# autonomousvision/connecting_the_dots

Measured on AMD Instinct MI355X. Metric: Mpix*disparities/s on 512x432x128 cost volume; disparity MAE vs ref, higher is better.
Workload: dtype f32

## Files before the change

### connecting_the_dots_amd/csrc/argmax_rerank.hip

```cpp
#include "ctd_internal.h"
#include "ctd_ncc_point.h"
#include "ctd_rank.h"
#include "ctd_tail.h"


namespace ctd {

constexpr int kScanBatch = 8;
template <int PX>
__global__ __launch_bounds__(256) __attribute__((amdgpu_waves_per_eu(5, 8))) void argmax_scan_kernel(const float* __restrict__ vol, int64_t* __restrict__ idx,
                                                          float* __restrict__ best, int D, long HW, int W,
                                                          int bs, float eps, long total_threads, WorkList work) {
  const long t = (long)blockIdx.x * blockDim.x + threadIdx.x;
  if (t >= total_threads) return;
  const long p0 = t * PX;
  const long f = p0 / HW, q0 = p0 - f * HW;
  const float* v = vol + f * D * HW + q0;
  const int w0 = (int)(q0 % W);
  float v0[PX], v1[PX];
  int i0[PX], dc[PX];
#pragma unroll
  for (int k = 0; k < PX; ++k) { v0[k] = -INFINITY; v1[k] = -INFINITY; i0[k] = 0; dc[k] = w0 + k + (bs - 1 - bs / 2); }
  constexpr int kBatch = kScanBatch;
  const bool wave_masks = __any(dc[0] < D - 1);
  for (int d0 = 0; d0 < D; d0 += kBatch) {
    float x[kBatch][PX];
#pragma unroll
    for (int u = 0; u < kBatch; ++u) {
      const float* src = v + (long)min(d0 + u, D - 1) * HW;
      if constexpr (PX == 4) {
        typedef float f4 __attribute__((ext_vector_type(4)));
        const f4 q = __builtin_nontemporal_load((const f4*)src);
        x[u][0] = q.x; x[u][1] = q.y; x[u][2] = q.z; x[u][3] = q.w;
      } else if constexpr (PX == 2) {
        typedef float f2 __attribute__((ext_vector_type(2)));
        const f2 q = __builtin_nontemporal_load((const f2*)src);
        x[u][0] = q.x; x[u][1] = q.y;
      } else {
        x[u][0] = __builtin_nontemporal_load(src);
      }
    }
    if (wave_masks || d0 + kBatch > D) {
#pragma unroll
      for (int u = 0; u < kBatch; ++u) {
        const int d = d0 + u;
#pragma unroll
        for (int k = 0; k < PX; ++k) {
          const float y = (d > dc[k] || d >= D) ? -INFINITY : x[u][k];
          v1[k] = __builtin_amdgcn_fmed3f(v0[k], v1[k], y);
          i0[k] = y > v0[k] ? d : i0[k];
          v0[k] = fmaxf(v0[k], y);
        }
      }
    } else {
#pragma unroll
      for (int u = 0; u < kBatch; ++u) {
#pragma unroll
        for (int k = 0; k < PX; ++k) {
          const float y = x[u][k];
          v1[k] = __builtin_amdgcn_fmed3f(v0[k], v1[k], y);
          i0[k] = y > v0[k] ? d0 + u : i0[k];
          v0[k] = fmaxf(v0[k], y);
        }
      }
    }
  }
#pragma unroll
  for (int k = 0; k < PX; ++k) {
    const bool hard = v1[k] >= v0[k] - eps;
    idx[p0 + k] = hard ? (int64_t)(-1 - i0[k]) : (int64_t)i0[k];
    if (best) best[p0 + k] = v0[k];
    if (hard) work.list[atomicAdd(work.counters, 1u)] = p0 + k;
  }
}

constexpr int kMaskWords = 8;

__device__ inline float wave_maxf(float v) {
#pragma unroll
  for (int o = 32; o > 0; o >>= 1) v = fmaxf(v, __shfl_xor(v, o));
  return v;
}

struct RunSource {
  const float* run_vals;
  const float* v1;
  int W1, xoff, per_frame;
};

template <int WORDS, bool VOL>
__device__ __forceinline__ void resolve_role(float* lds_resolve, const float* __restrict__ vol, const float* __restrict__ in0,
                                             const float* __restrict__ in1, long in1_frame_stride,
                                             int64_t* __restrict__ idx, float* __restrict__ best, int D, int H, int W, int bs,
                                             float eps, WorkList work, RunSource rsrc, unsigned role_block,
                                             unsigned n_role_blocks, unsigned waves_used = 4, unsigned* stamp = nullptr) {
  if ((threadIdx.x >> 6) >= waves_used) return;
  const int lane = threadIdx.x & 63;
  const int half = bs / 2, span = bs + D - 1;
  float* sA = lds_resolve + (threadIdx.x >> 6) * 2 * (bs * bs + bs * span);
  float* sB = sA + bs * bs;
  float* sAq = sB + bs * span;
  float* sBq = sAq + bs * bs;
  const float bs2f = (float)(bs * bs);
  const long HW = (long)H * W;
  unsigned seg_cnt[kWorkListParts];
  unsigned longest = 0;
#pragma unroll
  for (int k = 0; k < kWorkListParts; ++k) seg_cnt[k] = work.counters[min(k, work.parts - 1) * kWorkListStride];
#pragma unroll
  for (int k = 0; k < kWorkListParts; ++k) {
    if (k >= work.parts) seg_cnt[k] = 0u;
    longest = max(longest, seg_cnt[k]);
  }
  const unsigned n_slots = longest * (unsigned)work.parts;
  CTD_POST_STAMP_S(stamp, 1, longest);
  const unsigned n_waves = n_role_blocks * waves_used;
  for (unsigned slot = role_block * waves_used + (threadIdx.x >> 6); slot < n_slots; slot += n_waves) {
    const unsigned seg = slot & (unsigned)(work.parts - 1), entry = slot / (unsigned)work.parts;
    unsigned cnt = 0;
#pragma unroll
    for (int k = 0; k < kWorkListParts; ++k) cnt = seg == (unsigned)k ? seg_cnt[k] : cnt;
    if (entry >= cnt) continue;
    const long pj = work.list[(long)seg * work.seg_cap + entry];
    CTD_POST_STAMP_S(stamp, 2, pj);
    CTD_POST_STAMP_ITEM(stamp);
    const long fj = pj / HW, qj = pj - fj * HW;
    const int hj = (int)(qj / W), wj = (int)(qj - (long)hj * W);
    const float* v = VOL ? vol + fj * D * HW + qj : nullptr;
    const int d_clamped = wj + (bs - 1 - bs / 2);
    unsigned long long mask[WORDS];
    int n_cand = 0;
    float x[WORDS];
    bool run_listed = false;
    float rv = 0.f;
    if constexpr (VOL) {
      if (rsrc.run_vals && d_clamped < D) {
        const long z = rsrc.per_frame ? fj : 0;
        run_listed = rsrc.v1[(z * H + hj) * rsrc.W1 + (rsrc.xoff - (bs - 1 - bs / 2))] == 0.f;
        if (run_listed) rv = rsrc.run_vals[(fj * H + hj) * D + d_clamped];
      }
#pragma unroll
      for (int wd = 0; wd < WORDS; ++wd) {
        const int d = min(wd * 64 + lane, D - 1);
        x[wd] = v[(long)(rsrc.run_vals ? min(d, d_clamped) : d) * HW];
        if (run_listed && d >= d_clamped) x[wd] = rv;
      }
      CTD_POST_STAMP_V(stamp, 3, x[0]);
    }
    constexpr int kPreA = 2, kPreB = 20;
    const bool pre = !VOL && bs * bs <= 64 * kPreA && bs * span <= 64 * kPreB;
    const float* a = in0 + fj * HW;
    const float* b = in1 + fj * in1_frame_stride;
    float ta[kPreA], tb[kPreB];
    if (pre) {
#pragma unroll
      for (int k = 0; k < kPreA; ++k) {
        const int i = min(lane + 64 * k, bs * bs - 1);
        const int bh = i / bs, bw = i - bh * bs;
        ta[k] = a[(long)clampi(hj + bh - half, 0, H - 1) * W + clampi(wj + bw - half, 0, W - 1)];
      }
#pragma unroll
      for (int k = 0; k < kPreB; ++k) {
        const int i = min(lane + 64 * k, bs * span - 1);
        const int bh = i / span, c = i - bh * span;
        tb[k] = b[(long)clampi(hj + bh - half, 0, H - 1) * W + clampi(wj - half - (D - 1) + c, 0, W - 1)];
      }
    }
    if constexpr (VOL) {
      float m = -INFINITY;
#pragma unroll
      for (int wd = 0; wd < WORDS; ++wd)
        if (wd * 64 + lane < D && wd * 64 + lane <= d_clamped) m = fmaxf(m, x[wd]);
      m = wave_maxf(m);
      bool have_clamped = false;
#pragma unroll
      for (int wd = 0; wd < WORDS; ++wd) {
        unsigned long long bits = __ballot(wd * 64 + lane < D && x[wd] >= m - eps);
        const int c0 = d_clamped - wd * 64;
        if (c0 < 64) {
          const unsigned long long run = c0 <= 0 ? bits : bits & ~((1ull << c0) - 1ull);
          bits &= ~run;
          if (!have_clamped && run) {
            bits |= run & (0ull - run);
            have_clamped = true;
          }
        }
        mask[wd] = bits;
        n_cand += __popcll(bits);
      }
    } else {
#pragma unroll
      for (int wd = 0; wd < WORDS; ++wd) {
        const int last = min(D - 1, d_clamped) - wd * 64;
        mask[wd] = last < 0 ? 0ull : (last >= 63 ? ~0ull : ((1ull << (last + 1)) - 1ull));
        n_cand += __popcll(mask[wd]);
      }
    }
    float eb = 0.f;
    int ei = 0x7fffffff;
    const bool rescore = VOL ? n_cand > 1 : n_cand >= 1;
    if (rescore && pre) {
#pragma unroll
      for (int k = 0; k < kPreA; ++k)
        if (lane + 64 * k < bs * bs) {
          sA[lane + 64 * k] = ta[k];
          sAq[lane + 64 * k] = ta[k] / bs2f;
        }
#pragma unroll
      for (int k = 0; k < kPreB; ++k)
        if (lane + 64 * k < bs * span) {
          sB[lane + 64 * k] = tb[k];
          sBq[lane + 64 * k] = tb[k] / bs2f;
        }
    } else if (rescore) {
      for (int i = lane; i < bs * bs; i += 64) {
        const int bh = i / bs, bw = i - bh * bs;
        const float xa = a[(long)clampi(hj + bh - half, 0, H - 1) * W + clampi(wj + bw - half, 0, W - 1)];
        sA[i] = xa;
        sAq[i] = xa / bs2f;
      }
      constexpr int NB = 20;
      for (int i0 = lane; i0 < bs * span; i0 += 64 * NB) {
        float t[NB];
#pragma unroll
        for (int k = 0; k < NB; ++k) {
          const int i = min(i0 + 64 * k, bs * span - 1);
          const int bh = i / span, c = i - bh * span;
          t[k] = b[(long)clampi(hj + bh - half, 0, H - 1) * W + clampi(wj - half - (D - 1) + c, 0, W - 1)];
        }
#pragma unroll
        for (int k = 0; k < NB; ++k)
          if (i0 + 64 * k < bs * span) {
            sB[i0 + 64 * k] = t[k];
            sBq[i0 + 64 * k] = t[k] / bs2f;
          }
      }
    }
    CTD_POST_STAMP(stamp, 4);
    if (rescore) {
      for (int c0 = 0; c0 < n_cand; c0 += 64) {
        int my_d = -1, k = 0;
#pragma unroll
        for (int wd = 0; wd < WORDS; ++wd) {
          unsigned long long mj = mask[wd];
          if (k + __popcll(mj) <= c0 || k >= c0 + 64) { k += __popcll(mj); continue; }
          while (mj) {
            const int d = wd * 64 + __ffsll((long long)mj) - 1;
            mj &= mj - 1;
            if (k - c0 == lane) my_d = d;
            ++k;
          }
        }
        float e = -INFINITY;
        if (my_d >= 0) e = bs == 9 ? ncc_exact_point_lds_bs<9>(sA, sB, sAq, sBq, span, (D - 1) - my_d)
                                   : ncc_exact_point_lds(sA, sB, bs, span, (D - 1) - my_d);
        const float em = wave_maxf(e);
        const unsigned long long holders = __ballot(my_d >= 0 && e == em);
        const int dl = __shfl(my_d, holders ? __ffsll((long long)holders) - 1 : 0);
        if (ei == 0x7fffffff || em > eb) { eb = em; ei = dl; }
      }
    } else {
#pragma unroll
      for (int wd = 0; wd < WORDS; ++wd)
        if (mask[wd]) ei = min(ei, wd * 64 + __ffsll((long long)mask[wd]) - 1);
    }
    CTD_POST_STAMP_S(stamp, 5, ei);
    if (lane == 0) {
      idx[pj] = ei;
      if (best) {
        if constexpr (VOL) best[pj] = (run_listed && ei >= d_clamped) ? rv : v[(long)(rsrc.run_vals ? min(ei, d_clamped) : ei) * HW];
        else if (rescore) best[pj] = eb;
      }
    }
    CTD_POST_STAMP(stamp, 6);
    CTD_POST_STAMP(stamp, 9);
    stamp = nullptr;
  }
}

template <int WORDS, bool VOL>
__global__ __launch_bounds__(256) void argmax_resolve_kernel(const float* __restrict__ vol, const float* __restrict__ in0,
                                                             const float* __restrict__ in1, long in1_frame_stride,
                                                             int64_t* __restrict__ idx, float* __restrict__ best, int D,
                                                             int H, int W, int bs, float eps, WorkList work) {
  extern __shared__ float lds_dyn[];
  resolve_role<WORDS, VOL>(lds_dyn, vol, in0, in1, in1_frame_stride, idx, best, D, H, W, bs, eps, work,
                           RunSource{nullptr, nullptr, 0, 0, 0}, blockIdx.x, gridDim.x);
}

constexpr long kResolveBlocks = 1024;
constexpr unsigned kTailResolveWaves = 2;

template <int WORDS, bool VOL>
__global__ __launch_bounds__(256) void rank_tail_kernel(float* __restrict__ vol, const float* __restrict__ in0,
                                                        const float* __restrict__ in1, long in1_frame_stride,
                                                        int64_t* __restrict__ idx, float* __restrict__ best,
                                                        const unsigned char* __restrict__ flags, int frames, int D, int H,
                                                        int W, int bs, float eps, WorkList work, RunSource rsrc,
                                                        unsigned* __restrict__ counters,
                                                        const unsigned long long* __restrict__ run_rows,
                                                        const unsigned long long* __restrict__ flag_a,
                                                        const unsigned long long* __restrict__ flag_b, unsigned n_resolve,
                                                        unsigned n_runs, unsigned n_decode) {
  extern __shared__ float lds_dyn[];
  const unsigned n_pair = min(n_resolve, n_runs);
  unsigned role, rb;
  if (blockIdx.x < n_decode) { role = 2; rb = blockIdx.x; }
  else {
    const unsigned b = blockIdx.x - n_decode;
    if (b < 2 * n_pair) { role = b & 1; rb = b >> 1; }
    else { role = n_resolve > n_runs ? 0 : 1; rb = b - n_pair; }
  }
  if (blockIdx.x == 0 && threadIdx.x == 0) counters[0] = 0u;
  unsigned* stamp = CTD_POST_STAMP_SLOT(role);
  if (role == 0) {
    resolve_role<WORDS, VOL>(lds_dyn, vol, in0, in1, in1_frame_stride, idx, best, D, H, W, bs, eps, work, rsrc, rb, n_resolve,
                             kTailResolveWaves, stamp);
  } else if (role == 1) {
    if constexpr (VOL)
      runs_role(vol, rsrc.run_vals, counters, run_rows, rsrc.per_frame, 1, H, W, D, bs, (int)(rb >> 2), (int)(rb & 3), 4,
                (int*)lds_dyn, stamp);
  } else {
    decode_role((unsigned long long*)idx, best, flags, counters, flag_a, flag_b, rsrc.per_frame, frames, H, W, D,
                rb * 4 + (threadIdx.x >> 6), n_decode * 4, stamp);
  }
}


CTD_POST_STAMP_EXPORT(ctd_debug_read_tail_stamps)

template <bool VOL>
static int launch_resolve(const float* vol, const float* in0, const float* in1, long in1_frame_stride, int64_t* idx,
                          float* best, long total, int D, int H, int W, int bs, float eps, const WorkList& work,
                          hipStream_t stream) {
  const size_t lds = sizeof(float) * 4 * 2 * ((size_t)bs * bs + (size_t)bs * (bs + D - 1));
  if (lds > 160 * 1024) return CTD_ERR_UNSUPPORTED;
  const long chunks = (total + 255) / 256;
  auto resolve = D <= 128 ? argmax_resolve_kernel<2, VOL> : (D <= 256 ? argmax_resolve_kernel<4, VOL> : argmax_resolve_kernel<8, VOL>);
  if (lds > 64 * 1024)
    CTD_HIP_TRY(hipFuncSetAttribute((const void*)resolve, hipFuncAttributeMaxDynamicSharedMemorySize, (int)lds));
  hipLaunchKernelGGL(resolve, dim3((unsigned)(chunks < kResolveBlocks ? chunks : kResolveBlocks)), dim3(256), lds, stream, vol,
                     in0, in1, in1_frame_stride, idx, best, D, H, W, bs, eps, work);
  CTD_LAUNCH_CHECK();
  return CTD_OK;
}

template <bool VOL>
static int launch_tail(const RankPlan& rp, float* vol, const float* in0, const float* in1, long in1_frame_stride,
                       int64_t* idx, float* best, int frames, int D, int H, int W, int bs, hipStream_t stream) {
  size_t lds = sizeof(float) * kTailResolveWaves * 2 * ((size_t)bs * bs + (size_t)bs * (bs + D - 1));
  if (lds < sizeof(int) * (size_t)H) lds = sizeof(int) * (size_t)H;
  if (lds > 160 * 1024) return CTD_ERR_UNSUPPORTED;
  const long total = (long)frames * H * W;
  const long chunks = (total + 255) / 256;
  const unsigned n_resolve = rp.eps >= 0.f ? (unsigned)(chunks < kResolveBlocks ? chunks : kResolveBlocks) : 0u;
  const unsigned n_runs = VOL ? (unsigned)(frames * ceil_div(D, kRunPlanes)) * 4u : 0u;
  const unsigned n_decode = 128u;
  auto kern = D <= 128 ? rank_tail_kernel<2, VOL> : (D <= 256 ? rank_tail_kernel<4, VOL> : rank_tail_kernel<8, VOL>);
  if (lds > 64 * 1024)
    CTD_HIP_TRY(hipFuncSetAttribute((const void*)kern, hipFuncAttributeMaxDynamicSharedMemorySize, (int)lds));
  const RunSource rsrc = {rp.run_vals, rp.v1, rp.W1, rp.xoff, in1_frame_stride != 0 ? 1 : 0};
  hipLaunchKernelGGL(kern, dim3(n_resolve + n_runs + n_decode), dim3(256), lds, stream, vol, in0, in1, in1_frame_stride, idx,
                     best, rp.flags, frames, D, H, W, bs, rp.eps, rp.work, rsrc, rp.counters, rp.run_rows, rp.flag_a, rp.flag_b,
                     n_resolve,
                     n_runs, n_decode);
  CTD_LAUNCH_CHECK();
  return CTD_OK;
}

int rank_tail_f32(const RankPlan& rp, float* vol, const float* in0, const float* in1, long in1_frame_stride, int64_t* idx,
                  float* best, int frames, int D, int H, int W, int bs, hipStream_t stream) {
  return vol ? launch_tail<true>(rp, vol, in0, in1, in1_frame_stride, idx, best, frames, D, H, W, bs, stream)
             : launch_tail<false>(rp, nullptr, in0, in1, in1_frame_stride, idx, best, frames, D, H, W, bs, stream);
}

int argmax_rerank_f32(const float* vol, const float* in0, const float* in1, long in1_frame_stride, int64_t* idx,
                      float* best, int frames, int D, int H, int W, int bs, float eps, void* workspace,
                      size_t workspace_bytes, bool counter_cleared, hipStream_t stream) {
  if (D > kMaskWords * 64) return CTD_ERR_UNSUPPORTED;
  const long total = (long)frames * H * W;
  const long HW = (long)H * W;
  if (!workspace || workspace_bytes < 16 + sizeof(int64_t) * (size_t)total) return CTD_ERR_WORKSPACE;
  unsigned* n_hard = (unsigned*)workspace;
  const WorkList work = {n_hard, (int64_t*)((char*)workspace + 16), 1, W, total};
  if (!counter_cleared) CTD_HIP_TRY(hipMemsetAsync(n_hard, 0, 16, stream));
  const bool vec4 = W % 4 == 0 && ((uintptr_t)vol % 16) == 0;
  const int px = vec4 ? 4 : 1;
  if (px == 4)
    hipLaunchKernelGGL(argmax_scan_kernel<4>, dim3((unsigned)((total / 4 + 255) / 256)), dim3(256), 0, stream, vol,
                       idx, best, D, HW, W, bs, eps, total / 4, work);
  else
    hipLaunchKernelGGL(argmax_scan_kernel<1>, dim3((unsigned)((total + 255) / 256)), dim3(256), 0, stream, vol, idx,
                       best, D, HW, W, bs, eps, total, work);
  CTD_LAUNCH_CHECK();
  if (eps < 0.f) return CTD_OK;
  return launch_resolve<true>(vol, in0, in1, in1_frame_stride, idx, best, total, D, H, W, bs, eps, work, stream);
}

}
```

### connecting_the_dots_amd/csrc/ctd_ncc_point.h

```cpp
#ifndef CTD_NCC_POINT_H
#define CTD_NCC_POINT_H
#include "ctd_common.h"

namespace ctd {

__device__ inline float ncc_norm(float s0, float s1) {
  return (float)((double)sqrtf(s0 * s1) + 1e-8);
}
__device__ inline double ncc_norm(double s0, double s1) { return sqrt(s0 * s1) + 1e-8; }

__device__ inline float ncc_exact_term_lds(const float* sA, const float* sB, int bs, int span, int off) {
  const float bs2 = (float)(bs * bs);
  float mu0 = 0.f, mu1 = 0.f;
  for (int bh = 0; bh < bs; ++bh)
    for (int bw = 0; bw < bs; ++bw) {
      mu0 += sA[bh * bs + bw] / bs2;
      mu1 += sB[bh * span + bw + off] / bs2;
    }
  float s0 = 0.f, s1 = 0.f, dot = 0.f;
  for (int bh = 0; bh < bs; ++bh)
    for (int bw = 0; bw < bs; ++bw) {
      const float v0 = sA[bh * bs + bw] - mu0;
      const float v1 = sB[bh * span + bw + off] - mu1;
      dot += v0 * v1;
      s0 += v0 * v0;
      s1 += v1 * v1;
    }
  return dot / ncc_norm(s0, s1);
}
__device__ inline float ncc_exact_point_lds(const float* sA, const float* sB, int bs, int span, int off) {
  float val = 0.f;
  val += ncc_exact_term_lds(sA, sB, bs, span, off);
  return val;
}

template <int BS>
__device__ inline float ncc_exact_point_lds_bs(const float* sA, const float* sB, const float* sAq, const float* sBq,
                                               int span, int off) {
  float mu0 = 0.f, mu1 = 0.f;
  for (int bh = 0; bh < BS; ++bh) {
    float a[BS], b[BS];
#pragma unroll
    for (int bw = 0; bw < BS; ++bw) { a[bw] = sAq[bh * BS + bw]; b[bw] = sBq[bh * span + bw + off]; }
#pragma unroll
    for (int bw = 0; bw < BS; ++bw) {
      mu0 += a[bw];
      mu1 += b[bw];
    }
  }
  float s0 = 0.f, s1 = 0.f, dot = 0.f;
  for (int bh = 0; bh < BS; ++bh) {
    float a[BS], b[BS];
#pragma unroll
    for (int bw = 0; bw < BS; ++bw) { a[bw] = sA[bh * BS + bw]; b[bw] = sB[bh * span + bw + off]; }
#pragma unroll
    for (int bw = 0; bw < BS; ++bw) {
      const float v0 = a[bw] - mu0;
      const float v1 = b[bw] - mu1;
      dot += v0 * v1;
      s0 += v0 * v0;
      s1 += v1 * v1;
    }
  }
  float val = 0.f;
  val += dot / ncc_norm(s0, s1);
  return val;
}

}
#endif
```

Measured before the change: 1.034 million.

## Specialize bs=9 rerank path with halved LDS, two-pass means, occupancy-sized grid

Adds a bs=9 specialization of the resolve role. It stages window tiles in LDS once and runs the rescoring in two passes: a first pass computes the means from quotient-scaled values, then the raw values are restaged for the correlation sums. This halves the per-wave LDS footprint. The float divide by 81 is replaced with a reciprocal-multiply plus FMA correction, with a range guard and a fallback to true division. Work-item indices and the frame and row arithmetic are made wave-uniform via readfirstlane, which moves them to scalar registers. The tail kernel now uses 4 resolve waves with a launch-bounds occupancy hint and sizes its resolve grid from the queried occupancy. The rewrite adds complexity, and restaging between the passes costs extra LDS traffic.

```diff
diff --git a/connecting_the_dots_amd/csrc/argmax_rerank.hip b/connecting_the_dots_amd/csrc/argmax_rerank.hip
--- a/connecting_the_dots_amd/csrc/argmax_rerank.hip
+++ b/connecting_the_dots_amd/csrc/argmax_rerank.hip
@@ -1,5 +1,6 @@
 #include "ctd_internal.h"
 #include "ctd_ncc_point.h"
+#include "ctd_quot.h"
 #include "ctd_rank.h"
 #include "ctd_tail.h"
 
@@ -88,44 +89,65 @@
   int W1, xoff, per_frame;
 };
 
-template <int WORDS, bool VOL>
+constexpr int kResolveRegsA = 2, kResolveRegsB = 20;
+__host__ __device__ inline bool resolve_fits_regs(int bs, int D) {
+  return bs * bs <= 64 * kResolveRegsA && bs * (bs + D - 1) <= 64 * kResolveRegsB;
+}
+
+template <bool NARROW>
+__device__ __forceinline__ float frame_elem(const float* frame, int i) {
+  if constexpr (NARROW) return *(const float*)((const char*)frame + (unsigned)i * 4u);
+  else return frame[i];
+}
+
+inline bool resolve_b9(int bs, int D, int H, int W) { return bs == 9 && D >= 56 && D <= 128 && (long)H * W < (1L << 30); }
+
+__host__ __device__ inline int resolve_lds_floats(bool b9, int bs, int D) {
+  return b9 ? 64 * (kResolveRegsA + kResolveRegsB) : bs * bs + bs * (bs + D - 1);
+}
+
+template <int WORDS, bool VOL, bool B9>
 __device__ __forceinline__ void resolve_role(float* lds_resolve, const float* __restrict__ vol, const float* __restrict__ in0,
                                              const float* __restrict__ in1, long in1_frame_stride,
-                                             int64_t* __restrict__ idx, float* __restrict__ best, int D, int H, int W, int bs,
+                                             int64_t* __restrict__ idx, float* __restrict__ best, int D, int H, int W, int bs_rt,
                                              float eps, WorkList work, RunSource rsrc, unsigned role_block,
                                              unsigned n_role_blocks, unsigned waves_used = 4, unsigned* stamp = nullptr) {
   if ((threadIdx.x >> 6) >= waves_used) return;
   const int lane = threadIdx.x & 63;
+  const int bs = B9 ? 9 : bs_rt;
   const int half = bs / 2, span = bs + D - 1;
-  float* sA = lds_resolve + (threadIdx.x >> 6) * 2 * (bs * bs + bs * span);
-  float* sB = sA + bs * bs;
-  float* sAq = sB + bs * span;
-  float* sBq = sAq + bs * bs;
+  float* sA = lds_resolve + (threadIdx.x >> 6) * resolve_lds_floats(B9, bs, D);
+  float* sB = sA + (B9 ? 64 * kResolveRegsA : bs * bs);
   const float bs2f = (float)(bs * bs);
   const long HW = (long)H * W;
-  unsigned seg_cnt[kWorkListParts];
   unsigned longest = 0;
-#pragma unroll
-  for (int k = 0; k < kWorkListParts; ++k) seg_cnt[k] = work.counters[min(k, work.parts - 1) * kWorkListStride];
-#pragma unroll
-  for (int k = 0; k < kWorkListParts; ++k) {
-    if (k >= work.parts) seg_cnt[k] = 0u;
-    longest = max(longest, seg_cnt[k]);
+  {
+    unsigned seg_cnt[kWorkListParts];
+#pragma unroll
+    for (int k = 0; k < kWorkListParts; ++k) seg_cnt[k] = work.counters[min(k, work.parts - 1) * kWorkListStride];
+#pragma unroll
+    for (int k = 0; k < kWorkListParts; ++k)
+      if (k < work.parts) longest = max(longest, seg_cnt[k]);
   }
   const unsigned n_slots = longest * (unsigned)work.parts;
   CTD_POST_STAMP_S(stamp, 1, longest);
   const unsigned n_waves = n_role_blocks * waves_used;
   for (unsigned slot = role_block * waves_used + (threadIdx.x >> 6); slot < n_slots; slot += n_waves) {
     const unsigned seg = slot & (unsigned)(work.parts - 1), entry = slot / (unsigned)work.parts;
-    unsigned cnt = 0;
-#pragma unroll
-    for (int k = 0; k < kWorkListParts; ++k) cnt = seg == (unsigned)k ? seg_cnt[k] : cnt;
+    const unsigned cnt = work.counters[seg * kWorkListStride];
+    const long pj_lanes = work.list[(long)seg * work.seg_cap + entry];
+    const long pj = ((long)__builtin_amdgcn_readfirstlane((int)(pj_lanes >> 32)) << 32) |
+                    (long)(unsigned)__builtin_amdgcn_readfirstlane((int)pj_lanes);
     if (entry >= cnt) continue;
-    const long pj = work.list[(long)seg * work.seg_cap + entry];
     CTD_POST_STAMP_S(stamp, 2, pj);
     CTD_POST_STAMP_ITEM(stamp);
-    const long fj = pj / HW, qj = pj - fj * HW;
-    const int hj = (int)(qj / W), wj = (int)(qj - (long)hj * W);
+    long HW_j = HW;
+    int W_j = W;
+    asm volatile("" : "+s"(HW_j), "+s"(W_j));
+    const long fj = __builtin_amdgcn_readfirstlane((int)(pj / HW_j)), qj = pj - fj * HW;
+    const int hj = __builtin_amdgcn_readfirstlane((int)(qj / W_j)), wj = (int)(qj - (long)hj * W);
+    int ln = lane;
+    asm volatile("" : "+v"(ln));
     const float* v = VOL ? vol + fj * D * HW + qj : nullptr;
     const int d_clamped = wj + (bs - 1 - bs / 2);
     unsigned long long mask[WORDS];
@@ -141,31 +163,89 @@
       }
 #pragma unroll
       for (int wd = 0; wd < WORDS; ++wd) {
-        const int d = min(wd * 64 + lane, D - 1);
+        const int d = min(wd * 64 + ln, D - 1);
         x[wd] = v[(long)(rsrc.run_vals ? min(d, d_clamped) : d) * HW];
         if (run_listed && d >= d_clamped) x[wd] = rv;
       }
       CTD_POST_STAMP_V(stamp, 3, x[0]);
     }
-    constexpr int kPreA = 2, kPreB = 20;
-    const bool pre = !VOL && bs * bs <= 64 * kPreA && bs * span <= 64 * kPreB;
+    constexpr int kPreA = kResolveRegsA, kPreB = kResolveRegsB;
+    const bool one_trip = B9 || resolve_fits_regs(bs, D);
+    const bool pre = !VOL && one_trip;
     const float* a = in0 + fj * HW;
     const float* b = in1 + fj * in1_frame_stride;
     float ta[kPreA], tb[kPreB];
-    if (pre) {
+    auto load_rows = [&]() {
+      const int qa = 64 / bs, ra = 64 - qa * bs, qb = B9 ? 0 : 64 / span, rb = 64 - qb * span;
+      int bh = ln / bs, c = ln - bh * bs;
 #pragma unroll
       for (int k = 0; k < kPreA; ++k) {
-        const int i = min(lane + 64 * k, bs * bs - 1);
+        ta[k] = frame_elem<B9>(a, clampi(hj + bh - half, 0, H - 1) * W + clampi(wj + c - half, 0, W - 1));
+        bh += qa;
+        c += ra;
+        if (c >= bs) { c -= bs; ++bh; }
+      }
+      bh = B9 ? 0 : ln / span;
+      c = ln - bh * span;
+#pragma unroll
+      for (int k = 0; k < kPreB; ++k) {
+        tb[k] = frame_elem<B9>(b, clampi(hj + bh - half, 0, H - 1) * W + clampi(wj - half - (D - 1) + c, 0, W - 1));
+        bh += qb;
+        c += rb;
+        if (c >= span) { c -= span; ++bh; }
+      }
+    };
+    auto has_a = [&](int k) { return B9 || ln + 64 * k < bs * bs; };
+    auto has_b = [&](int k) { return B9 || ln + 64 * k < bs * span; };
+    auto store_rows_raw = [&]() {
+#pragma unroll
+      for (int k = 0; k < kPreA; ++k)
+        if (has_a(k)) sA[ln + 64 * k] = ta[k];
+#pragma unroll
+      for (int k = 0; k < kPreB; ++k)
+        if (has_b(k)) sB[ln + 64 * k] = tb[k];
+    };
+    auto store_rows_q81 = [&]() {
+      bool in_range = true;
+#pragma unroll
+      for (int k = 0; k < kPreA; ++k) {
+        in_range &= quot_in_range(ta[k]);
+        if (has_a(k)) sA[ln + 64 * k] = quot_const_unguarded<81>(ta[k]);
+      }
+#pragma unroll
+      for (int k = 0; k < kPreB; ++k) {
+        in_range &= quot_in_range(tb[k]);
+        if (has_b(k)) sB[ln + 64 * k] = quot_const_unguarded<81>(tb[k]);
+      }
+      if (!in_range) {
+#pragma unroll
+        for (int k = 0; k < kPreA; ++k)
+          if (has_a(k)) sA[ln + 64 * k] = ta[k] / 81.f;
+#pragma unroll
+        for (int k = 0; k < kPreB; ++k)
+          if (has_b(k)) sB[ln + 64 * k] = tb[k] / 81.f;
+      }
+    };
+    auto stage_rows = [&](bool quot) {
+      for (int i = ln; i < bs * bs; i += 64) {
         const int bh = i / bs, bw = i - bh * bs;
-        ta[k] = a[(long)clampi(hj + bh - half, 0, H - 1) * W + clampi(wj + bw - half, 0, W - 1)];
-      }
-#pragma unroll
-      for (int k = 0; k < kPreB; ++k) {
-        const int i = min(lane + 64 * k, bs * span - 1);
-        const int bh = i / span, c = i - bh * span;
-        tb[k] = b[(long)clampi(hj + bh - half, 0, H - 1) * W + clampi(wj - half - (D - 1) + c, 0, W - 1)];
-      }
-    }
+        const float xa = a[clampi(hj + bh - half, 0, H - 1) * W + clampi(wj + bw - half, 0, W - 1)];
+        sA[i] = quot ? quot_bs2(xa, bs, bs2f) : xa;
+      }
+      for (int i0 = ln; i0 < bs * span; i0 += 64 * kPreB) {
+        float t[kPreB];
+#pragma unroll
+        for (int k = 0; k < kPreB; ++k) {
+          const int i = min(i0 + 64 * k, bs * span - 1);
+          const int bh = i / span, c = i - bh * span;
+          t[k] = b[clampi(hj + bh - half, 0, H - 1) * W + clampi(wj - half - (D - 1) + c, 0, W - 1)];
+        }
+#pragma unroll
+        for (int k = 0; k < kPreB; ++k)
+          if (i0 + 64 * k < bs * span) sB[i0 + 64 * k] = quot ? quot_bs2(t[k], bs, bs2f) : t[k];
+      }
+    };
+    if (pre) load_rows();
     if constexpr (VOL) {
       float m = -INFINITY;
 #pragma unroll
@@ -199,46 +279,19 @@
     float eb = 0.f;
     int ei = 0x7fffffff;
     const bool rescore = VOL ? n_cand > 1 : n_cand >= 1;
-    if (rescore && pre) {
-#pragma unroll
-      for (int k = 0; k < kPreA; ++k)
-        if (lane + 64 * k < bs * bs) {
-          sA[lane + 64 * k] = ta[k];
-          sAq[lane + 64 * k] = ta[k] / bs2f;
-        }
-#pragma unroll
-      for (int k = 0; k < kPreB; ++k)
-        if (lane + 64 * k < bs * span) {
-          sB[lane + 64 * k] = tb[k];
-          sBq[lane + 64 * k] = tb[k] / bs2f;
-        }
-    } else if (rescore) {
-      for (int i = lane; i < bs * bs; i += 64) {
-        const int bh = i / bs, bw = i - bh * bs;
-        const float xa = a[(long)clampi(hj + bh - half, 0, H - 1) * W + clampi(wj + bw - half, 0, W - 1)];
-        sA[i] = xa;
-        sAq[i] = xa / bs2f;
-      }
-      constexpr int NB = 20;
-      for (int i0 = lane; i0 < bs * span; i0 += 64 * NB) {
-        float t[NB];
-#pragma unroll
-        for (int k = 0; k < NB; ++k) {
-          const int i = min(i0 + 64 * k, bs * span - 1);
-          const int bh = i / span, c = i - bh * span;
-          t[k] = b[(long)clampi(hj + bh - half, 0, H - 1) * W + clampi(wj - half - (D - 1) + c, 0, W - 1)];
-        }
-#pragma unroll
-        for (int k = 0; k < NB; ++k)
-          if (i0 + 64 * k < bs * span) {
-            sB[i0 + 64 * k] = t[k];
-            sBq[i0 + 64 * k] = t[k] / bs2f;
-          }
+    const bool two_pass = B9 || bs == 9;
+    if (rescore) {
+      if (one_trip) {
+        if (!pre) load_rows();
+        if (two_pass) store_rows_q81();
+        else store_rows_raw();
+      } else {
+        stage_rows(two_pass);
       }
     }
     CTD_POST_STAMP(stamp, 4);
     if (rescore) {
-      for (int c0 = 0; c0 < n_cand; c0 += 64) {
+      auto round_candidate = [&](int c0) {
         int my_d = -1, k = 0;
 #pragma unroll
         for (int wd = 0; wd < WORDS; ++wd) {
@@ -251,9 +304,38 @@
             ++k;
           }
         }
+        return my_d;
+      };
+      float mu0 = 0.f, mu1[WORDS];
+      if (two_pass) {
+        for (int c0 = 0, r = 0; c0 < n_cand; c0 += 64, ++r) {
+          const int my_d = round_candidate(c0);
+          if (my_d >= 0) {
+            float m0, m1;
+            ncc_point_means_lds<9>(sA, sB, span, (D - 1) - my_d, m0, m1);
+            mu0 = m0;
+#pragma unroll
+            for (int k = 0; k < WORDS; ++k)
+              if (k == r) mu1[k] = m1;
+          }
+        }
+        if (one_trip) store_rows_raw();
+        else stage_rows(false);
+      }
+      for (int c0 = 0, r = 0; c0 < n_cand; c0 += 64, ++r) {
+        const int my_d = round_candidate(c0);
         float e = -INFINITY;
-        if (my_d >= 0) e = bs == 9 ? ncc_exact_point_lds_bs<9>(sA, sB, sAq, sBq, span, (D - 1) - my_d)
-                                   : ncc_exact_point_lds(sA, sB, bs, span, (D - 1) - my_d);
+        if (my_d >= 0) {
+          if (two_pass) {
+            float m1 = 0.f;
+#pragma unroll
+            for (int k = 0; k < WORDS; ++k)
+              if (k == r) m1 = mu1[k];
+            e = ncc_point_chains_lds<9>(sA, sB, span, (D - 1) - my_d, mu0, m1);
+          } else {
+            e = ncc_exact_point_lds(sA, sB, bs, span, (D - 1) - my_d);
+          }
+        }
         const float em = wave_maxf(e);
         const unsigned long long holders = __ballot(my_d >= 0 && e == em);
         const int dl = __shfl(my_d, holders ? __ffsll((long long)holders) - 1 : 0);
@@ -278,21 +360,22 @@
   }
 }
 
-template <int WORDS, bool VOL>
+template <int WORDS, bool VOL, bool B9>
 __global__ __launch_bounds__(256) void argmax_resolve_kernel(const float* __restrict__ vol, const float* __restrict__ in0,
                                                              const float* __restrict__ in1, long in1_frame_stride,
                                                              int64_t* __restrict__ idx, float* __restrict__ best, int D,
                                                              int H, int W, int bs, float eps, WorkList work) {
   extern __shared__ float lds_dyn[];
-  resolve_role<WORDS, VOL>(lds_dyn, vol, in0, in1, in1_frame_stride, idx, best, D, H, W, bs, eps, work,
-                           RunSource{nullptr, nullptr, 0, 0, 0}, blockIdx.x, gridDim.x);
+  resolve_role<WORDS, VOL, B9>(lds_dyn, vol, in0, in1, in1_frame_stride, idx, best, D, H, W, bs, eps, work,
+                               RunSource{nullptr, nullptr, 0, 0, 0}, blockIdx.x, gridDim.x);
 }
 
 constexpr long kResolveBlocks = 1024;
-constexpr unsigned kTailResolveWaves = 2;
-
-template <int WORDS, bool VOL>
-__global__ __launch_bounds__(256) void rank_tail_kernel(float* __restrict__ vol, const float* __restrict__ in0,
+constexpr unsigned kTailResolveWaves = 4;
+constexpr long kTailResolveBlocks = 512;
+
+template <int WORDS, bool VOL, bool B9>
+__global__ __launch_bounds__(256, B9 ? 7 : 1) void rank_tail_kernel(float* __restrict__ vol, const float* __restrict__ in0,
                                                         const float* __restrict__ in1, long in1_frame_stride,
                                                         int64_t* __restrict__ idx, float* __restrict__ best,
                                                         const unsigned char* __restrict__ flags, int frames, int D, int H,
@@ -314,8 +397,8 @@
   if (blockIdx.x == 0 && threadIdx.x == 0) counters[0] = 0u;
   unsigned* stamp = CTD_POST_STAMP_SLOT(role);
   if (role == 0) {
-    resolve_role<WORDS, VOL>(lds_dyn, vol, in0, in1, in1_frame_stride, idx, best, D, H, W, bs, eps, work, rsrc, rb, n_resolve,
-                             kTailResolveWaves, stamp);
+    resolve_role<WORDS, VOL, B9>(lds_dyn, vol, in0, in1, in1_frame_stride, idx, best, D, H, W, bs, eps, work, rsrc, rb,
+                                 n_resolve, kTailResolveWaves, stamp);
   } else if (role == 1) {
     if constexpr (VOL)
       runs_role(vol, rsrc.run_vals, counters, run_rows, rsrc.per_frame, 1, H, W, D, bs, (int)(rb >> 2), (int)(rb & 3), 4,
@@ -333,10 +416,13 @@
 static int launch_resolve(const float* vol, const float* in0, const float* in1, long in1_frame_stride, int64_t* idx,
                           float* best, long total, int D, int H, int W, int bs, float eps, const WorkList& work,
                           hipStream_t stream) {
-  const size_t lds = sizeof(float) * 4 * 2 * ((size_t)bs * bs + (size_t)bs * (bs + D - 1));
+  const bool b9 = resolve_b9(bs, D, H, W);
+  const size_t lds = sizeof(float) * 4 * (size_t)resolve_lds_floats(b9, bs, D);
   if (lds > 160 * 1024) return CTD_ERR_UNSUPPORTED;
   const long chunks = (total + 255) / 256;
-  auto resolve = D <= 128 ? argmax_resolve_kernel<2, VOL> : (D <= 256 ? argmax_resolve_kernel<4, VOL> : argmax_resolve_kernel<8, VOL>);
+  auto resolve = b9 ? argmax_resolve_kernel<2, VOL, true>
+                    : (D <= 128 ? argmax_resolve_kernel<2, VOL, false>
+                                : (D <= 256 ? argmax_resolve_kernel<4, VOL, false> : argmax_resolve_kernel<8, VOL, false>));
   if (lds > 64 * 1024)
     CTD_HIP_TRY(hipFuncSetAttribute((const void*)resolve, hipFuncAttributeMaxDynamicSharedMemorySize, (int)lds));
   hipLaunchKernelGGL(resolve, dim3((unsigned)(chunks < kResolveBlocks ? chunks : kResolveBlocks)), dim3(256), lds, stream, vol,
@@ -348,17 +434,35 @@
 template <bool VOL>
 static int launch_tail(const RankPlan& rp, float* vol, const float* in0, const float* in1, long in1_frame_stride,
                        int64_t* idx, float* best, int frames, int D, int H, int W, int bs, hipStream_t stream) {
-  size_t lds = sizeof(float) * kTailResolveWaves * 2 * ((size_t)bs * bs + (size_t)bs * (bs + D - 1));
+  const bool b9 = resolve_b9(bs, D, H, W);
+  size_t lds = sizeof(float) * kTailResolveWaves * (size_t)resolve_lds_floats(b9, bs, D);
   if (lds < sizeof(int) * (size_t)H) lds = sizeof(int) * (size_t)H;
   if (lds > 160 * 1024) return CTD_ERR_UNSUPPORTED;
   const long total = (long)frames * H * W;
   const long chunks = (total + 255) / 256;
-  const unsigned n_resolve = rp.eps >= 0.f ? (unsigned)(chunks < kResolveBlocks ? chunks : kResolveBlocks) : 0u;
   const unsigned n_runs = VOL ? (unsigned)(frames * ceil_div(D, kRunPlanes)) * 4u : 0u;
   const unsigned n_decode = 128u;
-  auto kern = D <= 128 ? rank_tail_kernel<2, VOL> : (D <= 256 ? rank_tail_kernel<4, VOL> : rank_tail_kernel<8, VOL>);
+  const int words = b9 ? 3 : (D <= 128 ? 0 : (D <= 256 ? 1 : 2));
+  auto kern = b9 ? rank_tail_kernel<2, VOL, true>
+                 : (D <= 128 ? rank_tail_kernel<2, VOL, false>
+                             : (D <= 256 ? rank_tail_kernel<4, VOL, false> : rank_tail_kernel<8, VOL, false>));
   if (lds > 64 * 1024)
     CTD_HIP_TRY(hipFuncSetAttribute((const void*)kern, hipFuncAttributeMaxDynamicSharedMemorySize, (int)lds));
+  static struct { size_t lds; int dev, per_cu; } occ[2][4] = {};
+  int dev = 0;
+  (void)hipGetDevice(&dev);
+  auto& oc = occ[VOL ? 1 : 0][words];
+  if (oc.per_cu == 0 || oc.lds != lds || oc.dev != dev) {
+    int n = 0;
+    if (hipOccupancyMaxActiveBlocksPerMultiprocessor(&n, (const void*)kern, 256, lds) != hipSuccess || n < 1) n = 1;
+    oc = {lds, dev, n};
+  }
+  const long n_cu = device_cu_count();
+  long room = (long)oc.per_cu * n_cu - (long)n_runs - (long)n_decode;
+  if (room < n_cu) room = n_cu;
+  long want = (chunks + 1) / 2;
+  if (want > kTailResolveBlocks) want = kTailResolveBlocks;
+  const unsigned n_resolve = rp.eps >= 0.f ? (unsigned)(want < room ? want : room) : 0u;
   const RunSource rsrc = {rp.run_vals, rp.v1, rp.W1, rp.xoff, in1_frame_stride != 0 ? 1 : 0};
   hipLaunchKernelGGL(kern, dim3(n_resolve + n_runs + n_decode), dim3(256), lds, stream, vol, in0, in1, in1_frame_stride, idx,
                      best, rp.flags, frames, D, H, W, bs, rp.eps, rp.work, rsrc, rp.counters, rp.run_rows, rp.flag_a, rp.flag_b,
diff --git a/connecting_the_dots_amd/csrc/ctd_ncc_point.h b/connecting_the_dots_amd/csrc/ctd_ncc_point.h
--- a/connecting_the_dots_amd/csrc/ctd_ncc_point.h
+++ b/connecting_the_dots_amd/csrc/ctd_ncc_point.h
@@ -35,9 +35,10 @@
 }
 
 template <int BS>
-__device__ inline float ncc_exact_point_lds_bs(const float* sA, const float* sB, const float* sAq, const float* sBq,
-                                               int span, int off) {
+__device__ inline void ncc_point_means_lds(const float* sAq, const float* sBq, int span, int off, float& mu0_out,
+                                           float& mu1_out) {
   float mu0 = 0.f, mu1 = 0.f;
+#pragma unroll 1
   for (int bh = 0; bh < BS; ++bh) {
     float a[BS], b[BS];
 #pragma unroll
@@ -48,7 +49,14 @@
       mu1 += b[bw];
     }
   }
+  mu0_out = mu0;
+  mu1_out = mu1;
+}
+
+template <int BS>
+__device__ inline float ncc_point_chains_lds(const float* sA, const float* sB, int span, int off, float mu0, float mu1) {
   float s0 = 0.f, s1 = 0.f, dot = 0.f;
+#pragma unroll 3
   for (int bh = 0; bh < BS; ++bh) {
     float a[BS], b[BS];
 #pragma unroll
diff --git a/connecting_the_dots_amd/csrc/ctd_quot.h b/connecting_the_dots_amd/csrc/ctd_quot.h
--- /dev/null
+++ b/connecting_the_dots_amd/csrc/ctd_quot.h
@@ -0,0 +1,40 @@
+#ifndef CTD_QUOT_H
+#define CTD_QUOT_H
+#include <math.h>
+
+#if defined(__HIPCC__) || defined(__CUDACC__)
+#define CTD_QUOT_HD __host__ __device__
+#else
+#define CTD_QUOT_HD
+#endif
+
+namespace ctd {
+
+template <int C> struct QuotProven { static constexpr bool value = false; };
+template <> struct QuotProven<81> { static constexpr bool value = true; };
+
+constexpr unsigned kQuotExpLo = 127u - 96u, kQuotExpHi = 127u + 96u - 1u;
+
+CTD_QUOT_HD inline bool quot_in_range(float x) {
+  const unsigned e = (__builtin_bit_cast(unsigned, x) >> 23) & 0xFFu;
+  return e - kQuotExpLo <= kQuotExpHi - kQuotExpLo;
+}
+
+template <int C>
+CTD_QUOT_HD inline float quot_const_unguarded(float x) {
+  static_assert(QuotProven<C>::value, "no exhaustive proof for this divisor: use the division");
+  constexpr float c = (float)C, r = 1.f / (float)C;
+  const float q0 = x * r;
+  const float e = fmaf(-c, q0, x);
+  return fmaf(e, r, q0);
+}
+
+template <int C>
+CTD_QUOT_HD inline float quot_const(float x) {
+  return quot_in_range(x) ? quot_const_unguarded<C>(x) : x / (float)C;
+}
+
+CTD_QUOT_HD inline float quot_bs2(float x, int bs, float n) { return bs == 9 ? quot_const<81>(x) : x / n; }
+
+}
+#endif
```

Result: no change. 1.038 million, median of 3 (+0.4%).
